# ramanathanlab/distllm

Hardware: NVIDIA H100
Metric: embedded chunks/sec @512-tok (higher is better)
Workload: dtype bf16

## Files before the change

distllm_b200/csrc/attention.cuh:

```cuda
#pragma once

#include "common.cuh"

namespace b2e {

constexpr int AT_KC = 64;
constexpr float AT_MASKED = -3.0e38f;

template <int D, int V>
struct AtCfg {
  static constexpr int COLS = D < 64 ? D : 64;
  static constexpr int ROW_BYTES = 2 * COLS;
  static constexpr int BOX = 64 * ROW_BYTES;
  static constexpr int NB = D / COLS;
  static constexpr int NWG = (V & 64) ? 4 : 2;
  static constexpr int QT = 64 * NWG;
  static constexpr int THREADS = 128 * NWG + (NWG == 4 ? 128 : 32);
  static constexpr int CONSUMER_REGS = 112, PRODUCER_REGS = 24;
  static constexpr int STAGES = D == 128 ? 3 : 4;
  static constexpr int Q_BYTES = NWG * NB * BOX;
  static constexpr int STAGE_BYTES = 2 * NB * BOX;
  static_assert(D == 32 || D == 64 || D == 128, "head_dim");
  static constexpr int BAR = Q_BYTES + STAGES * STAGE_BYTES;
  static constexpr int SMEM_BYTES = BAR + 256 + 1024;
  static_assert(SMEM_BYTES <= 232448, "shared memory");
};

__device__ long long* g_att_clock = nullptr;

__device__ __forceinline__ float poly_exp2(float x) {
  x = fmaxf(x, -126.0f);
  const float n = rintf(x);
  const float f = x - n;
  float p = fmaf(f, 9.6181291e-3f, 5.5504109e-2f);
  p = fmaf(f, p, 2.4022651e-1f);
  p = fmaf(f, p, 6.9314718e-1f);
  p = fmaf(f, p, 1.0f);
  return __int_as_float(__float_as_int(p) + (static_cast<int>(n) << 23));
}

template <int ROW_BYTES>
__device__ __forceinline__ uint64_t at_box_desc(uint32_t saddr) {
  if constexpr (ROW_BYTES == 128) return make_smem_desc_sw128(saddr);
  else return make_smem_desc_sw64(saddr);
}

__global__ void attn_prep_kernel(const int64_t* __restrict__ mask, float* __restrict__ bias,
                                 int* __restrict__ kv_chunks, int* __restrict__ plain_chunks, int B, int S,
                                 int S_pad) {
  const int b = blockIdx.x * (blockDim.x >> 5) + (threadIdx.x >> 5);
  if (b >= B) return;
  const int lane = threadIdx.x & 31;
  int last = 0;
  int first_off = S_pad;
  for (int j = lane; j < S_pad; j += 32) {
    float v = -INFINITY;
    bool on = false;
    if (j < S) {
      on = mask[static_cast<size_t>(b) * S + j] != 0;
      v = on ? 0.0f : AT_MASKED;
      if (on) last = j + 1;
    }
    if (!on) first_off = min(first_off, j);
    bias[static_cast<size_t>(b) * S_pad + j] = v;
  }
#pragma unroll
  for (int o = 16; o > 0; o >>= 1) {
    last = max(last, __shfl_xor_sync(0xffffffffu, last, o));
    first_off = min(first_off, __shfl_xor_sync(0xffffffffu, first_off, o));
  }
  if (lane == 0) {
    kv_chunks[b] = last > 0 ? (last + AT_KC - 1) / AT_KC : S_pad / AT_KC;
    plain_chunks[b] = first_off / AT_KC;
  }
}

template <int D, int MODE, int V>
__global__ void __launch_bounds__(AtCfg<D, V>::THREADS, 1)
attention_kernel(const __grid_constant__ CUtensorMap tm, const __grid_constant__ CUtensorMap tm_ctx,
                 const float* __restrict__ bias, const int* __restrict__ kv_chunks,
                 const int* __restrict__ plain_chunks, int B, int S, int S_pad, int heads, int kv_heads, int window,
                 float scale_log2e, const int* __restrict__ seq_cu, const int* __restrict__ seq_len,
                 h16* __restrict__ ctx) {
  using Cfg = AtCfg<D, V>;
  constexpr int NB = Cfg::NB;
  constexpr int COLS = Cfg::COLS, BOX = Cfg::BOX, RB = Cfg::ROW_BYTES;
  constexpr int NWG = Cfg::NWG;
  constexpr int POLY = (V >> 2) & 3;
  constexpr bool EPI_ROLE = (V & 128) != 0;
  constexpr bool STAMPS = (V & 256) != 0;
  static_assert(MODE == 0 || (V & ~(64 | 128)) == 0, "windowed / causal attention: warpgroups and epilogue role only");
  const int h = blockIdx.x % heads;
  const int b = (blockIdx.x / heads) % B;
  const int tile = static_cast<int>(gridDim.x / (heads * B)) - 1 - static_cast<int>(blockIdx.x / (heads * B));
  const int row0 = seq_cu != nullptr ? __ldg(seq_cu + b) : b * S;
  const int len = seq_len != nullptr ? __ldg(seq_len + b) : S;
  const int q0 = tile * Cfg::QT;
  if (q0 >= len) return;
  const int kvc = __ldg(kv_chunks + b);
  const int np = (V & 1) ? __ldg(plain_chunks + b) : 0;
  int lo = 0, hi = kvc;
  if (MODE == 1) {
    lo = max(0, q0 - window) / AT_KC;
    hi = min(kvc, (q0 + Cfg::QT - 1 + window) / AT_KC + 1);
  } else if (MODE == 2) {
    lo = window > 0 ? max(0, q0 - window + 1) / AT_KC : 0;
    hi = min(kvc, (q0 + Cfg::QT - 1) / AT_KC + 1);
  }
  if (lo >= hi) lo = hi - 1;

  extern __shared__ uint8_t smem_raw[];
  const uint32_t sb = (smem_u32(smem_raw) + 1023u) & ~1023u;
  const uint32_t q_bar = sb + Cfg::BAR;
  const uint32_t full_bar = q_bar + 8;
  const uint32_t empty_bar = full_bar + 8u * Cfg::STAGES;
  const uint32_t out_bar = empty_bar + 8u * Cfg::STAGES;
  const int warp = threadIdx.x >> 5;
  const int kvh = h / (heads / kv_heads);
  const int qcol = h * D, kcol = (heads + kvh) * D, vcol = (heads + kv_heads + kvh) * D;

  if (threadIdx.x == 0) {
    mbar_init(q_bar, 1);
    for (int s = 0; s < Cfg::STAGES; ++s) {
      mbar_init(full_bar + 8u * s, 1);
      mbar_init(empty_bar + 8u * s, NWG);
    }
    for (int w = 0; w < NWG; ++w) mbar_init(out_bar + 8u * w, 1);
    mbar_fence_init();
  }
  __syncthreads();

  if (warp >= 4 * NWG) {
    if constexpr (NWG == 4) asm volatile("setmaxnreg.dec.sync.aligned.u32 %0;" ::"n"(Cfg::PRODUCER_REGS));
    if (warp == 4 * NWG && elect_one()) {
      tma_prefetch_desc(&tm);
      mbar_expect_tx(q_bar, Cfg::Q_BYTES);
#pragma unroll
      for (int w = 0; w < NWG; ++w)
#pragma unroll
        for (int x = 0; x < NB; ++x)
          tma_load_2d(sb + (w * NB + x) * BOX, &tm, q_bar, qcol + COLS * x, row0 + q0 + 64 * w);
      int stage = 0;
      uint32_t phase = 0;
      for (int c = lo; c < hi; ++c) {
        mbar_wait(empty_bar + 8u * stage, phase ^ 1u);
        const uint32_t fb = full_bar + 8u * stage;
        const uint32_t dst = sb + Cfg::Q_BYTES + stage * Cfg::STAGE_BYTES;
        mbar_expect_tx(fb, Cfg::STAGE_BYTES);
#pragma unroll
        for (int x = 0; x < NB; ++x) {
          tma_load_2d(dst + x * BOX, &tm, fb, kcol + COLS * x, row0 + c * AT_KC);
          tma_load_2d(dst + (NB + x) * BOX, &tm, fb, vcol + COLS * x, row0 + c * AT_KC);
        }
        if (++stage == Cfg::STAGES) { stage = 0; phase ^= 1u; }
      }
      if constexpr (EPI_ROLE) {
        for (int w = 0; w < NWG; ++w) {
          mbar_wait(out_bar + 8u * w, 0);
          if (q0 + 64 * w + 64 > len) continue;
#pragma unroll
          for (int x = 0; x < NB; ++x)
            tma_store_2d(&tm_ctx, sb + (w * NB + x) * BOX, h * D + COLS * x, row0 + q0 + 64 * w);
        }
        tma_store_commit();
        tma_store_wait_all();
      }
    }
    return;
  }

  if constexpr (NWG == 4) asm volatile("setmaxnreg.inc.sync.aligned.u32 %0;" ::"n"(Cfg::CONSUMER_REGS));
  const int wg = warp >> 2;
  const int t = threadIdx.x & 127;
  const int quad = t & 3;
  const int qr = q0 + 64 * wg + 16 * (t >> 5) + ((t & 31) >> 2);
  const float* brow = bias + static_cast<size_t>(b) * S_pad;
  const uint32_t q_addr = sb + wg * NB * BOX;
  long long* clk = nullptr;
  int n_stamp = 0;
  if (STAMPS && blockIdx.x == 0 && threadIdx.x == 0) clk = g_att_clock;

  constexpr int OG = COLS / 8;
  float o[NB][4 * OG];
#pragma unroll
  for (int x = 0; x < NB; ++x)
#pragma unroll
    for (int i = 0; i < 4 * OG; ++i) o[x][i] = 0.0f;
  float m[2] = {-INFINITY, -INFINITY}, l[2] = {0.0f, 0.0f};

  mbar_wait(q_bar, 0);
  int stage = 0;
  uint32_t phase = 0;
  for (int c = lo; c < hi; ++c) {
    mbar_wait(full_bar + 8u * stage, phase);
    const uint32_t k_addr = sb + Cfg::Q_BYTES + stage * Cfg::STAGE_BYTES;
    const uint32_t v_addr = k_addr + NB * BOX;
    float s[32];
#pragma unroll
    for (int i = 0; i < 32; ++i) s[i] = 0.0f;
    wgmma_fence();
    constexpr int KB = COLS / 16;
#pragma unroll
    for (int kk = 0; kk < D / 16; ++kk)
      wgmma_64x64_ss<0>(s, at_box_desc<RB>(q_addr + (kk / KB) * BOX) + 2u * (kk % KB),
                        at_box_desc<RB>(k_addr + (kk / KB) * BOX) + 2u * (kk % KB), kk != 0);
    wgmma_commit();
    wgmma_wait<0>();
    reg_fence(s);
    if (STAMPS && clk != nullptr && n_stamp < 256) {
      clk[n_stamp] = clock64();
      clk[256 + n_stamp++] = 2 * c + 1;
    }

    const int kbase = c * AT_KC + 2 * quad;
    const bool plain = MODE == 0 && (V & 1) && c < np;
#pragma unroll
    for (int j = 0; j < 8; ++j) {
      const float2 bz = plain ? make_float2(0.0f, 0.0f) : *reinterpret_cast<const float2*>(brow + kbase + 8 * j);
#pragma unroll
      for (int e = 0; e < 4; ++e) {
        const int key = kbase + 8 * j + (e & 1);
        const int q = qr + 8 * (e >> 1);
        float x = fmaf(s[4 * j + e], scale_log2e, (e & 1) ? bz.y : bz.x);
        if (MODE == 1 && abs(q - key) > window) x = AT_MASKED;
        if (MODE == 2 && (key > q || (window > 0 && q - key >= window))) x = AT_MASKED;
        s[4 * j + e] = x;
      }
    }
    float alpha[2];
#pragma unroll
    for (int hf = 0; hf < 2; ++hf) {
      float mx = m[hf];
#pragma unroll
      for (int j = 0; j < 8; ++j) mx = fmaxf(mx, fmaxf(s[4 * j + 2 * hf], s[4 * j + 2 * hf + 1]));
      mx = fmaxf(mx, __shfl_xor_sync(0xffffffffu, mx, 1));
      mx = fmaxf(mx, __shfl_xor_sync(0xffffffffu, mx, 2));
      alpha[hf] = fast_exp2(m[hf] - mx);
      m[hf] = mx;
    }
    uint32_t p[4][4];
    float rs[2] = {0.0f, 0.0f};
#pragma unroll
    for (int j = 0; j < 8; ++j) {
#pragma unroll
      for (int hf = 0; hf < 2; ++hf) {
        const float x0 = s[4 * j + 2 * hf] - m[hf], x1 = s[4 * j + 2 * hf + 1] - m[hf];
        const int k0 = (2 * (j & 1) + hf) * 2;
        const float p0 = (k0 % 4) < POLY ? poly_exp2(x0) : fast_exp2(x0);
        const float p1 = ((k0 + 1) % 4) < POLY ? poly_exp2(x1) : fast_exp2(x1);
        rs[hf] += p0 + p1;
        p[j >> 1][(j & 1) * 2 + hf] = pack_h16x2(p0, p1);
      }
    }
#pragma unroll
    for (int hf = 0; hf < 2; ++hf) l[hf] = l[hf] * alpha[hf] + rs[hf];
#pragma unroll
    for (int x = 0; x < NB; ++x)
#pragma unroll
      for (int j = 0; j < OG; ++j) {
        o[x][4 * j + 0] *= alpha[0];
        o[x][4 * j + 1] *= alpha[0];
        o[x][4 * j + 2] *= alpha[1];
        o[x][4 * j + 3] *= alpha[1];
      }

#pragma unroll
    for (int x = 0; x < NB; ++x) reg_fence(o[x]);
    wgmma_fence();
#pragma unroll
    for (int kc = 0; kc < 4; ++kc)
#pragma unroll
      for (int x = 0; x < NB; ++x) {
        if constexpr (COLS == 64) wgmma_64x64_rs_tb(o[x], p[kc], make_smem_desc_sw128(v_addr + x * BOX + kc * 16 * 128));
        else wgmma_64x32_rs_tb(o[x], p[kc], make_smem_desc_sw64(v_addr + x * BOX + kc * 16 * 64));
      }
    wgmma_commit();
    wgmma_wait<0>();
#pragma unroll
    for (int x = 0; x < NB; ++x) reg_fence(o[x]);
    if (STAMPS && clk != nullptr && n_stamp < 256) {
      clk[n_stamp] = clock64();
      clk[256 + n_stamp++] = 2 * c + 2;
    }
    if (t == 0) mbar_arrive(empty_bar + 8u * stage);
    if (++stage == Cfg::STAGES) { stage = 0; phase ^= 1u; }
  }

  const bool staged = EPI_ROLE && q0 + 64 * wg + 64 <= len;
#pragma unroll
  for (int hf = 0; hf < 2; ++hf) {
    float tot = l[hf];
    tot += __shfl_xor_sync(0xffffffffu, tot, 1);
    tot += __shfl_xor_sync(0xffffffffu, tot, 2);
    const float inv = 1.0f / tot;
    const int q = qr + 8 * hf;
    if (staged) {
      const int r = q - q0 - 64 * wg;
      const int swz = RB == 128 ? (r & 7) : ((r >> 1) & 3);
#pragma unroll
      for (int x = 0; x < NB; ++x)
#pragma unroll
        for (int j = 0; j < OG; ++j) {
          const uint32_t off = r * RB + ((j ^ swz) << 4) + 4 * quad;
          *reinterpret_cast<uint32_t*>(smem_raw + (q_addr - smem_u32(smem_raw)) + x * BOX + off) =
              pack_h16x2(o[x][4 * j + 2 * hf] * inv, o[x][4 * j + 2 * hf + 1] * inv);
        }
      continue;
    }
    if (q >= len) continue;
    h16* orow = ctx + static_cast<size_t>(row0 + q) * (heads * D) + h * D + 2 * quad;
#pragma unroll
    for (int x = 0; x < NB; ++x)
#pragma unroll
      for (int j = 0; j < OG; ++j)
        *reinterpret_cast<uint32_t*>(orow + COLS * x + 8 * j) =
            pack_h16x2(o[x][4 * j + 2 * hf] * inv, o[x][4 * j + 2 * hf + 1] * inv);
  }
  if constexpr (EPI_ROLE) {
    fence_proxy_async_smem();
    asm volatile("bar.sync %0, 128;" ::"r"(1 + wg) : "memory");
    if (t == 0) mbar_arrive(out_bar + 8u * wg);
  }
}

}
```

distllm_b200/csrc/b2e_api.cu:

```cuda
#include "../../include/b2e.h"
#include "../../include/b2e_debug.h"

#include <cuda.h>
#include <cuda_runtime.h>

#include <cstdarg>
#include <cstdio>
#include <cstdlib>
#include <cstring>
#include <string>
#include <utility>
#include <vector>

#include "attention.cuh"
#include "binsearch.cuh"
#include "common.cuh"
#include "gemm.cuh"
#include "mistral_ops.cuh"
#include "pack.cuh"
#include "rowops.cuh"
#include "topk.cuh"
#include "topk_tc.cuh"

using namespace b2e;
// ... 178 lines not shown
  CUtensorMap tm;
  const float* absmax = nullptr;
  int bn = GEMM_BN;
};

int make_gemm_w(GemmW* w, const void* base, const float* absmax, uint64_t rows, uint64_t cols, int epi) {
  w->absmax = absmax;
  w->bn = gemm_bn((int)rows, epi, absmax != nullptr);
  return absmax ? make_tmap_codes(&w->tm, base, rows, cols / 2) : make_tmap_h16(&w->tm, base, rows, cols, w->bn);
}

template <int EPI>
int launch_gemm_epi(const CUtensorMap& ta, const GemmW& wb, void* out, const float* bias,
                    const h16* resid, int M, int N, int K, cudaStream_t st, const int* m_dev) {
  auto kern = gemm_h16_wgmma_kernel<EPI>;
  int smem = GemmPlan<false>::SMEM_BYTES;
  if (N % wb.bn != 0) return fail(B2E_ERR_INVALID, "gemm: N=%d is not a multiple of its W map's tile width %d", N, wb.bn);
  if (wb.absmax) {
    kern = gemm_h16_wgmma_kernel<EPI, false, true>;
    smem = GemmPlan<true>::SMEM_BYTES;
  } else if (wb.bn == 192) {
    if constexpr (epi_is_glu(EPI)) {
      return fail(B2E_ERR_INVALID, "gemm: the gated epilogues run 128-wide tiles only");
    } else {
      kern = gemm_h16_wgmma_kernel<EPI, false, false, 192>;
      smem = GemmPlan<false, 192>::SMEM_BYTES;
      if constexpr (EPI == EPI_BIAS || EPI == EPI_BIAS_GELU)
        if (g_gemm_profiling) kern = gemm_h16_wgmma_kernel<EPI, true, false, 192>;
    }
  } else if constexpr (EPI == EPI_BIAS || EPI == EPI_BIAS_GELU) {
    if (g_gemm_profiling) kern = gemm_h16_wgmma_kernel<EPI, true>;
  }
  int rc = ensure_smem_attr(kern, smem);
  if (rc) return rc;
  DeviceInfo dev;
  if ((rc = current_device_info(&dev))) return rc;
  const long long tiles = (long long)(N / wb.bn) * ((M + GEMM_BM - 1) / GEMM_BM);
  if (tiles > 0x7fffffffLL) return fail(B2E_ERR_INVALID, "gemm: %lld output tiles exceed one grid", tiles);
  CUtensorMap tm_out;
  if ((rc = make_tmap_h16(&tm_out, out, M, epi_is_glu(EPI) ? N / 2 : N, GEMM_BM))) return rc;
  const unsigned grid = (unsigned)(tiles < dev.sms ? tiles : dev.sms);
  kern<<<grid, GEMM_THREADS, smem, st>>>(ta, wb.tm, tm_out, static_cast<h16*>(out), bias, resid, M, N, K, m_dev,
                                         wb.absmax);
  CUDA_TRY(cudaGetLastError());
  return B2E_OK;
}

int launch_gemm(const CUtensorMap& ta, const GemmW& tb, void* out, const float* bias,
                const void* resid, int M, int N, int K, int epi, cudaStream_t st, const int* m_dev = nullptr) {
  const h16* r = static_cast<const h16*>(resid);
  switch (epi) {
    case B2E_EPI_BIAS: return launch_gemm_epi<EPI_BIAS>(ta, tb, out, bias, r, M, N, K, st, m_dev);
    case B2E_EPI_BIAS_GELU: return launch_gemm_epi<EPI_BIAS_GELU>(ta, tb, out, bias, r, M, N, K, st, m_dev);
    case B2E_EPI_BIAS_RESID: return launch_gemm_epi<EPI_BIAS_RESID>(ta, tb, out, bias, r, M, N, K, st, m_dev);
    case B2E_EPI_SWIGLU: return launch_gemm_epi<EPI_SWIGLU>(ta, tb, out, bias, r, M, N, K, st, m_dev);
    case B2E_EPI_GEGLU: return launch_gemm_epi<EPI_GEGLU>(ta, tb, out, bias, r, M, N, K, st, m_dev);
  }
  return fail(B2E_ERR_INVALID, "unknown epilogue %d", epi);
}

template <typename T>
struct DevBuf {
  T* p = nullptr;
  size_t cap = 0;
  operator T*() const { return p; }
  int grow(size_t n, uint64_t& gen, bool zero = false) {
    if (n <= cap) return B2E_OK;
    ++gen;
    release();
    CUDA_TRY(cudaMalloc(&p, n * sizeof(T)));
    if (zero) CUDA_TRY(cudaMemset(p, 0, n * sizeof(T)));
    cap = n;
    return B2E_OK;
  }
  void release() {
    cudaFree(p);
    p = nullptr;
    cap = 0;
  }
};

struct DeviceScratch {
  int device = -1;
  uint64_t gen = 0;
};

template <typename Scratch>
int follow_device(Scratch& s) {
  int dev = 0;
  CUDA_TRY(cudaGetDevice(&dev));
  if (dev != s.device) {
    s.release();
    s.device = dev;
    ++s.gen;
  }
  return B2E_OK;
}

struct AttnScratch : DeviceScratch {
  DevBuf<float> bias;
  DevBuf<int> kv_chunks;
  DevBuf<int> plain_chunks;
  int ensure(int B, int S_pad) {
    int rc;
    if ((rc = follow_device(*this)) || (rc = bias.grow((size_t)B * S_pad, gen)) || (rc = kv_chunks.grow(B, gen)) ||
        (rc = plain_chunks.grow(B, gen)))
      return rc;
    return B2E_OK;
  }
  void release() {
    bias.release();
    kv_chunks.release();
    plain_chunks.release();
  }
};

inline int attn_s_pad(int S) { return (S + AT_KC - 1) / AT_KC * AT_KC; }

int attention_prepare(AttnScratch& sc, const int64_t* mask, int B, int S, cudaStream_t st) {
  int rc;
  const int S_pad = attn_s_pad(S);
  if ((rc = sc.ensure(B, S_pad))) return rc;
  attn_prep_kernel<<<(B + 7) / 8, 256, 0, st>>>(mask, sc.bias, sc.kv_chunks, sc.plain_chunks, B, S, S_pad);
  CUDA_TRY(cudaGetLastError());
  return B2E_OK;
}

struct SeqLayout {
  const int* cu = nullptr;
  const int* len = nullptr;
  const int* t_real = nullptr;
  const int* tok_src = nullptr;
};

struct PackBuffers : DeviceScratch {
  DevBuf<int> len_raw, ok, len;
  DevBuf<int> cu;
  DevBuf<int> t_real;
  DevBuf<int> src;
  int ensure(int B, size_t tokens) {
    int rc;
    if ((rc = follow_device(*this)) || (rc = len_raw.grow(B, gen)) || (rc = ok.grow(B, gen)) ||
        (rc = len.grow(B, gen)) || (rc = cu.grow((size_t)B + 1, gen)) || (rc = t_real.grow(2, gen)) ||
        (rc = src.grow(tokens, gen)))
      return rc;
    return B2E_OK;
  }
  void release() {
    len_raw.release(); ok.release(); len.release(); cu.release(); t_real.release(); src.release();
  }
};

template <int D, int MODE, int V>
int launch_attention_kernel(const CUtensorMap& tm, const AttnScratch& sc, void* ctx, int B, int S, int heads,
                            int kv_heads, int window, cudaStream_t st, const SeqLayout& lay) {
  using Cfg = AtCfg<D, V>;
  auto kern = attention_kernel<D, MODE, V>;
  int rc = ensure_smem_attr(kern, Cfg::SMEM_BYTES);
  if (rc) return rc;
  CUtensorMap tm_ctx = {};
  if ((V & 128) && (rc = make_tmap_h16(&tm_ctx, ctx, (uint64_t)B * S, (uint64_t)heads * D, 64, Cfg::COLS))) return rc;
  const float scale_log2e = 1.4426950408889634f / sqrtf(static_cast<float>(D));
  const long long ctas = (long long)heads * B * ((S + Cfg::QT - 1) / Cfg::QT);
  if (ctas > 0x7fffffffLL)
    return fail(B2E_ERR_INVALID, "attention: %lld CTAs (heads=%d B=%d S=%d) exceed one grid", ctas, heads, B, S);
  kern<<<(unsigned)ctas, Cfg::THREADS, Cfg::SMEM_BYTES, st>>>(tm, tm_ctx, sc.bias, sc.kv_chunks, sc.plain_chunks, B, S,
                                                    attn_s_pad(S), heads, kv_heads, window, scale_log2e, lay.cu,
                                                    lay.len, static_cast<h16*>(ctx));
  CUDA_TRY(cudaGetLastError());
  return B2E_OK;
}

constexpr int AT_DEFAULT_VARIANT = 193;
int g_att3_variant = -1;
inline int att3_variant() {
  if (g_att3_variant < 0) {
    const char* e = getenv("B2E_ATT3");
    g_att3_variant = e ? atoi(e) : AT_DEFAULT_VARIANT;
  }
  return g_att3_variant;
}

int launch_attention(const CUtensorMap& tkv, const AttnScratch& sc, void* ctx, int B, int S, int heads,
                     cudaStream_t st, int window = 0, const SeqLayout& lay = SeqLayout()) {
  const int v = att3_variant();
#define B2E_ATT(MODE, V) launch_attention_kernel<64, MODE, V>(tkv, sc, ctx, B, S, heads, heads, window, st, lay)
  if (window > 0) {
    switch (v & 192) {
      case 0: return B2E_ATT(1, 0);
      case 64: return B2E_ATT(1, 64);
      case 128: return B2E_ATT(1, 128);
      case 192: return B2E_ATT(1, 192);
    }
    return fail(B2E_ERR_INVALID, "windowed attention: variant %d has no instantiation (bits 6-7 of the variant pick "
                "0, 64, 128 or 192)", v);
  }
  switch (v) {
    case 0: return B2E_ATT(0, 0);
    case 1: return B2E_ATT(0, 1);
    case 5: return B2E_ATT(0, 5);
    case 64: return B2E_ATT(0, 64);
    case 65: return B2E_ATT(0, 65);
    case 69: return B2E_ATT(0, 69);
    case 193: return B2E_ATT(0, 193);
    case 261: return B2E_ATT(0, 261);
    case 321: return B2E_ATT(0, 321);
  }
#undef B2E_ATT
  return fail(B2E_ERR_INVALID, "attention variant %d is not instantiated (0,1,5,64,65,69,193,261,321)", v);
}

int launch_attention_causal_d128(const void* qkv, AttnScratch& sc, void* ctx, int B, int S, int heads,
                                 int kv_heads, int window, cudaStream_t st, const SeqLayout& lay = SeqLayout()) {
  CUtensorMap tm;
  const int rc = make_tmap_h16(&tm, qkv, (uint64_t)B * S, (uint64_t)(heads + 2 * kv_heads) * 128, AT_KC);
  if (rc) return rc;
  return launch_attention_kernel<128, 2, 0>(tm, sc, ctx, B, S, heads, kv_heads, window, st, lay);
}

constexpr int AT_D32_VARIANT = 1;

int launch_attention_bidir(const CUtensorMap& tqkv, const AttnScratch& sc, void* ctx, int B, int S, int heads,
                           int head_dim, cudaStream_t st, const SeqLayout& lay = SeqLayout()) {
  if (head_dim == 32)
    return launch_attention_kernel<32, 0, AT_D32_VARIANT>(tqkv, sc, ctx, B, S, heads, heads, 0, st, lay);
  return launch_attention(tqkv, sc, ctx, B, S, heads, st, 0, lay);
}

#define DISPATCH_H(H, CALL)                                         \
  switch (H) {                                                      \
    case 256: { constexpr int HW = 256; CALL; break; }              \
    case 384: { constexpr int HW = 384; CALL; break; }              \
    case 512: { constexpr int HW = 512; CALL; break; }              \
    case 640: { constexpr int HW = 640; CALL; break; }              \
    case 768: { constexpr int HW = 768; CALL; break; }              \
    case 1024: { constexpr int HW = 1024; CALL; break; }            \
    case 1280: { constexpr int HW = 1280; CALL; break; }            \
    case 2048: { constexpr int HW = 2048; CALL; break; }            \
    case 2560: { constexpr int HW = 2560; CALL; break; }            \
    case 4096: { constexpr int HW = 4096; CALL; break; }            \
    default: return fail(B2E_ERR_INVALID, "hidden size %d not supported (need 256*{1,2,3,4,5,8,10,16}, 384 or 640)", (H)); \
  }

inline int row_blocks(int rows) { return (rows + ROW_WARPS - 1) / ROW_WARPS; }

int check_h(int H) {
  if (H == 384 || H == 640) return B2E_OK;
  if (H % 256 != 0) return fail(B2E_ERR_INVALID, "hidden size %d must be a multiple of 256, or 384 or 640", H);
  switch (H / 256) {
    case 1: case 2: case 3: case 4: case 5: case 8: case 10: case 16: return B2E_OK;
  }
  return fail(B2E_ERR_UNSUPPORTED, "hidden size %d not supported (built: 256 x {1,2,3,4,5,8,10,16}, 384, 640)", H);
}

struct PoolScratch : DeviceScratch {
  DevBuf<int> seq_len;
  DevBuf<int> kill;
  DevBuf<int> idx;
  DevBuf<float> w;
  DevBuf<float> count;
  DevBuf<float> part;
  int ensure(int B, int S, size_t part_elems) {
    int rc;
    if ((rc = follow_device(*this)) || (rc = seq_len.grow(B, gen)) || (rc = kill.grow(S, gen)) ||
        (rc = idx.grow(B, gen)) || (rc = w.grow((size_t)B * S, gen)) || (rc = count.grow(B, gen)) ||
        (rc = part.grow(part_elems, gen)))
      return rc;
    return B2E_OK;
  }
  void release() {
    seq_len.release(); kill.release(); idx.release(); w.release(); count.release(); part.release();
  }
};

inline int pool_nsplit(int S) {
  int n = (S + 63) / 64;
  return n < 1 ? 1 : (n > 16 ? 16 : n);
}

int launch_pool_weights(PoolScratch& ps, int64_t* mask, int B, int S, int pool_kind, int mutate,
                        cudaStream_t st) {
  seq_len_kernel<<<(B + 7) / 8, 256, 0, st>>>(mask, ps.seq_len, B, S);
  CUDA_TRY(cudaMemsetAsync(ps.kill, 0, sizeof(int) * S, st));
  kill_columns_kernel<<<(B + 255) / 256, 256, 0, st>>>(ps.seq_len, ps.kill, B, S);
  pool_weights_kernel<<<(B + 7) / 8, 256, 0, st>>>(mask, ps.seq_len, ps.kill, ps.w, ps.count, B, S,
                                                    pool_kind == B2E_POOL_MEAN_REF ? 1 : 0, mutate);
  CUDA_TRY(cudaGetLastError());
  return B2E_OK;
}

int launch_finalize(PoolScratch& ps, float* out, int B, int H, int nsplit, int l2, int round_mode,
                    cudaStream_t st) {
  pool_finalize_kernel<<<B, 256, (H + 32) * sizeof(float), st>>>(ps.part, ps.count, out, H, nsplit,
                                                                 l2, round_mode);
  CUDA_TRY(cudaGetLastError());
  return B2E_OK;
}

struct DeviceGuard {
  int prev = -1;
  DeviceGuard() {
    if (cudaGetDevice(&prev) != cudaSuccess) {
      cudaGetLastError();
      prev = -1;
    }
  }
  ~DeviceGuard() {
    if (prev >= 0) cudaSetDevice(prev);
  }
};

thread_local PoolScratch g_pool_scratch;
thread_local AttnScratch g_attn_scratch;
thread_local PackBuffers g_pack_scratch;

}

inline bool is_decoder(int arch) { return arch == B2E_ARCH_MISTRAL || arch == B2E_ARCH_QWEN3; }

namespace {
enum FinalNorm {
  NORM_POST_LN,
  NORM_ADD_LN,
  NORM_ADD_RMS,
};

using TrunkFn = int (*)(B2EEncoder* e, const int64_t* ids, const int64_t* mask, const int64_t* types, int B, int S,
                        cudaStream_t st, const SeqLayout& lay);

struct Family {
  int lead, stride;
  int wqkv, wo, w1, w2;
  bool w1_gated;
  int w1_epi;
  FinalNorm norm;
  int norm_g, norm_b;
  TrunkFn trunk;
};
const Family* family(int arch);
}

struct B2EEncoder {
  B2EModelDesc desc;
  const Family* fam = nullptr;
  int full_layers = 0;
  std::vector<const void*> w;
  int device = 0;
  int sms = 0;
  DevBuf<h16> hidden, qkv, ctx, tmp, ffn;
  DevBuf<float> xres, tok_scale;
  PoolScratch pool;
  AttnScratch attn;
  PackBuffers pack;
  std::vector<GemmW> tm_wqkv, tm_wo, tm_w1, tm_w2;
  DevBuf<int64_t> stage_in;
  DevBuf<float> stage_out;
  cudaStream_t own_stream = nullptr;
  float *rope_cos = nullptr, *rope_sin = nullptr;
  float *rope_cos2 = nullptr, *rope_sin2 = nullptr;

  const void* slot(int l, int k) const { return w[fam->lead + fam->stride * l + k]; }
  const float* final_norm(int k) const {
// ... 1255 lines not shown
```

Before: 5007.

## Add ping-pong warpgroup attention kernel for head_dim 64 and make it default

Adds a new FlashAttention-3 style kernel for head_dim 64. Two consumer warpgroups each own 128 query rows and alternate wgmma issue through named barriers. Inside each turn, the S=QK^T GEMM for the next chunk overlaps the PV GEMM for the previous chunk, so softmax runs while the tensor cores stay busy. It uses 8 KV stages, 240 consumer registers and a TMA store epilogue, and it becomes the default variant (705). The risks are register pressure and barrier ordering in the ping-pong schedule, and the larger per-CTA query tile may lower parallelism at short sequence lengths.

Measured after the change: 5050, median of 6. About the same (+0.9%).

```diff
diff --git a/distllm_b200/csrc/attention.cuh b/distllm_b200/csrc/attention.cuh
--- a/distllm_b200/csrc/attention.cuh
+++ b/distllm_b200/csrc/attention.cuh
@@ -323,4 +323,266 @@
   }
 }
 
-}
+constexpr int AT_BAR_TURN = 1, AT_BAR_EPI = 3;
+
+struct AtPingPongCfg {
+  static constexpr int COLS = 64;
+  static constexpr int BOX = 64 * 2 * COLS;
+  static constexpr int NWG = 2;
+  static constexpr int QT = 128 * NWG;
+  static constexpr int THREADS = 128 * NWG + 128;
+  static constexpr int CONSUMER_REGS = 240, PRODUCER_REGS = 24;
+  static constexpr int STAGES = 8;
+  static constexpr int Q_BYTES = 2 * NWG * BOX;
+  static constexpr int STAGE_BYTES = 2 * BOX;
+  static constexpr int BAR = Q_BYTES + STAGES * STAGE_BYTES;
+  static constexpr int SMEM_BYTES = BAR + 256 + 1024;
+  static_assert(SMEM_BYTES <= 232448, "shared memory");
+};
+
+__device__ __forceinline__ void at_softmax_block(float (&s)[32], const float2 (&bz)[8], float scale_log2e,
+                                                 float (&m)[2], float (&l)[2], float (&alpha)[2],
+                                                 uint32_t (&p)[4][4]) {
+#pragma unroll
+  for (int j = 0; j < 8; ++j)
+#pragma unroll
+    for (int e = 0; e < 4; ++e) s[4 * j + e] = fmaf(s[4 * j + e], scale_log2e, (e & 1) ? bz[j].y : bz[j].x);
+#pragma unroll
+  for (int hf = 0; hf < 2; ++hf) {
+    float mx = m[hf];
+#pragma unroll
+    for (int j = 0; j < 8; ++j) mx = fmaxf(mx, fmaxf(s[4 * j + 2 * hf], s[4 * j + 2 * hf + 1]));
+    mx = fmaxf(mx, __shfl_xor_sync(0xffffffffu, mx, 1));
+    mx = fmaxf(mx, __shfl_xor_sync(0xffffffffu, mx, 2));
+    alpha[hf] = fast_exp2(m[hf] - mx);
+    m[hf] = mx;
+  }
+  float rs[2] = {0.0f, 0.0f};
+#pragma unroll
+  for (int j = 0; j < 8; ++j)
+#pragma unroll
+    for (int hf = 0; hf < 2; ++hf) {
+      const float p0 = fast_exp2(s[4 * j + 2 * hf] - m[hf]), p1 = fast_exp2(s[4 * j + 2 * hf + 1] - m[hf]);
+      rs[hf] += p0 + p1;
+      p[j >> 1][(j & 1) * 2 + hf] = pack_h16x2(p0, p1);
+    }
+#pragma unroll
+  for (int hf = 0; hf < 2; ++hf) l[hf] = l[hf] * alpha[hf] + rs[hf];
+}
+
+template <int V>
+__global__ void __launch_bounds__(AtPingPongCfg::THREADS, 1)
+pingpong_attention_kernel(const __grid_constant__ CUtensorMap tm, const __grid_constant__ CUtensorMap tm_ctx,
+                          const float* __restrict__ bias, const int* __restrict__ kv_chunks,
+                          const int* __restrict__ plain_chunks, int B, int S, int S_pad, int heads, int kv_heads,
+                          int window, float scale_log2e, const int* __restrict__ seq_cu,
+                          const int* __restrict__ seq_len, h16* __restrict__ ctx) {
+  using Cfg = AtPingPongCfg;
+  constexpr int BOX = Cfg::BOX, NWG = Cfg::NWG, D = 64;
+  static_assert(V & 512, "ping-pong variants have bit 9 set");
+  const int tiles = static_cast<int>(gridDim.x / (heads * B));
+  const int tile = static_cast<int>(blockIdx.x % tiles);
+  const int h = static_cast<int>(blockIdx.x / tiles) % heads;
+  const int b = static_cast<int>(blockIdx.x / (tiles * heads));
+  const int row0 = seq_cu != nullptr ? __ldg(seq_cu + b) : b * S;
+  const int len = seq_len != nullptr ? __ldg(seq_len + b) : S;
+  const int q0 = tile * Cfg::QT;
+  if (q0 >= len) return;
+  const int lo = 0, hi = __ldg(kv_chunks + b);
+  const int np = (V & 1) ? __ldg(plain_chunks + b) : 0;
+
+  extern __shared__ uint8_t smem_raw[];
+  const uint32_t sb = (smem_u32(smem_raw) + 1023u) & ~1023u;
+  const uint32_t q_bar = sb + Cfg::BAR;
+  const uint32_t full_bar = q_bar + 8;
+  const uint32_t empty_bar = full_bar + 8u * Cfg::STAGES;
+  const int warp = threadIdx.x >> 5;
+  const int kvh = h / (heads / kv_heads);
+  const int qcol = h * D, kcol = (heads + kvh) * D, vcol = (heads + kv_heads + kvh) * D;
+
+  if (threadIdx.x == 0) {
+    mbar_init(q_bar, 1);
+    for (int s = 0; s < Cfg::STAGES; ++s) {
+      mbar_init(full_bar + 8u * s, 1);
+      mbar_init(empty_bar + 8u * s, NWG);
+    }
+    mbar_fence_init();
+  }
+  __syncthreads();
+
+  if (warp >= 4 * NWG) {
+    asm volatile("setmaxnreg.dec.sync.aligned.u32 %0;" ::"n"(Cfg::PRODUCER_REGS));
+    if (warp == 4 * NWG && elect_one()) {
+      tma_prefetch_desc(&tm);
+      mbar_expect_tx(q_bar, Cfg::Q_BYTES);
+#pragma unroll
+      for (int x = 0; x < 2 * NWG; ++x) tma_load_2d(sb + x * BOX, &tm, q_bar, qcol, row0 + q0 + 64 * x);
+      int stage = 0;
+      uint32_t phase = 0;
+      for (int c = lo; c < hi; ++c) {
+        mbar_wait(empty_bar + 8u * stage, phase ^ 1u);
+        const uint32_t fb = full_bar + 8u * stage;
+        const uint32_t dst = sb + Cfg::Q_BYTES + stage * Cfg::STAGE_BYTES;
+        mbar_expect_tx(fb, Cfg::STAGE_BYTES);
+        tma_load_2d(dst, &tm, fb, kcol, row0 + c * AT_KC);
+        tma_load_2d(dst + BOX, &tm, fb, vcol, row0 + c * AT_KC);
+        if (++stage == Cfg::STAGES) { stage = 0; phase ^= 1u; }
+      }
+    }
+    return;
+  }
+
+  asm volatile("setmaxnreg.inc.sync.aligned.u32 %0;" ::"n"(Cfg::CONSUMER_REGS));
+  const int wg = warp >> 2;
+  const int t = threadIdx.x & 127;
+  const int quad = t & 3;
+  const int r_lo = 16 * (t >> 5) + ((t & 31) >> 2);
+  const int wrow = q0 + 128 * wg;
+  const float* brow = bias + static_cast<size_t>(b) * S_pad;
+  const uint32_t q_addr = sb + 2 * wg * BOX;
+
+  float o[2][32], s[2][32];
+#pragma unroll
+  for (int i = 0; i < 32; ++i) o[0][i] = o[1][i] = s[0][i] = s[1][i] = 0.0f;
+  float m[2][2] = {{-INFINITY, -INFINITY}, {-INFINITY, -INFINITY}}, l[2][2] = {{0.0f, 0.0f}, {0.0f, 0.0f}};
+  uint32_t pa[2][4][4], pb[2][4][4];
+
+  auto issue_s = [&](uint32_t k_addr) {
+#pragma unroll
+    for (int kk = 0; kk < D / 16; ++kk)
+#pragma unroll
+      for (int bl = 0; bl < 2; ++bl)
+        wgmma_64x64_ss<0>(s[bl], make_smem_desc_sw128(q_addr + bl * BOX) + 2u * kk,
+                          make_smem_desc_sw128(k_addr) + 2u * kk, kk != 0);
+  };
+  auto issue_pv = [&](const uint32_t (&p)[2][4][4], uint32_t v_addr) {
+#pragma unroll
+    for (int kc = 0; kc < 4; ++kc)
+#pragma unroll
+      for (int bl = 0; bl < 2; ++bl) wgmma_64x64_rs_tb(o[bl], p[bl][kc], make_smem_desc_sw128(v_addr + kc * 16 * 128));
+  };
+  auto load_bias = [&](int c, float2 (&bz)[8]) {
+    const bool plain = (V & 1) && c < np;
+    const int kbase = c * AT_KC + 2 * quad;
+#pragma unroll
+    for (int j = 0; j < 8; ++j)
+      bz[j] = plain ? make_float2(0.0f, 0.0f) : *reinterpret_cast<const float2*>(brow + kbase + 8 * j);
+  };
+  const uint32_t kv0 = sb + Cfg::Q_BYTES;
+
+  mbar_wait(q_bar, 0);
+  float alpha[2][2];
+  {
+    float2 bz[8];
+    load_bias(lo, bz);
+    mbar_wait(full_bar, 0);
+    if (wg == 1) named_bar_sync(AT_BAR_TURN + 1, 256);
+    wgmma_fence();
+    issue_s(kv0);
+    wgmma_commit();
+    named_bar_arrive(AT_BAR_TURN + (wg ^ 1), 256);
+    wgmma_wait<0>();
+    reg_fence(s[0]);
+    reg_fence(s[1]);
+#pragma unroll
+    for (int bl = 0; bl < 2; ++bl) at_softmax_block(s[bl], bz, scale_log2e, m[bl], l[bl], alpha[bl], pa[bl]);
+  }
+  static_assert(Cfg::STAGES > 1, "chunk lo + 1 is in stage 1");
+  int stage = 1, prev = 0;
+  uint32_t phase = 0;
+  auto turn = [&](int c, const uint32_t (&in)[2][4][4], uint32_t (&out)[2][4][4]) {
+    float2 bz[8];
+    load_bias(c, bz);
+    mbar_wait(full_bar + 8u * stage, phase);
+    named_bar_sync(AT_BAR_TURN + wg, 256);
+    reg_fence(o[0]);
+    reg_fence(o[1]);
+    wgmma_fence();
+    issue_s(kv0 + stage * Cfg::STAGE_BYTES);
+    wgmma_commit();
+    issue_pv(in, kv0 + prev * Cfg::STAGE_BYTES + BOX);
+    wgmma_commit();
+    named_bar_arrive(AT_BAR_TURN + (wg ^ 1), 256);
+    wgmma_wait<1>();
+    reg_fence(s[0]);
+    reg_fence(s[1]);
+#pragma unroll
+    for (int bl = 0; bl < 2; ++bl) at_softmax_block(s[bl], bz, scale_log2e, m[bl], l[bl], alpha[bl], out[bl]);
+    wgmma_wait<0>();
+    reg_fence(o[0]);
+    reg_fence(o[1]);
+    if (t == 0) mbar_arrive(empty_bar + 8u * prev);
+#pragma unroll
+    for (int bl = 0; bl < 2; ++bl)
+#pragma unroll
+      for (int j = 0; j < 8; ++j) {
+        o[bl][4 * j + 0] *= alpha[bl][0];
+        o[bl][4 * j + 1] *= alpha[bl][0];
+        o[bl][4 * j + 2] *= alpha[bl][1];
+        o[bl][4 * j + 3] *= alpha[bl][1];
+      }
+    prev = stage;
+    if (++stage == Cfg::STAGES) { stage = 0; phase ^= 1u; }
+  };
+  auto last_turn = [&](const uint32_t (&in)[2][4][4]) {
+    named_bar_sync(AT_BAR_TURN + wg, 256);
+    reg_fence(o[0]);
+    reg_fence(o[1]);
+    wgmma_fence();
+    issue_pv(in, kv0 + prev * Cfg::STAGE_BYTES + BOX);
+    wgmma_commit();
+    if (wg == 0) named_bar_arrive(AT_BAR_TURN + 1, 256);
+    wgmma_wait<0>();
+    reg_fence(o[0]);
+    reg_fence(o[1]);
+  };
+  int c = lo + 1;
+  for (; c + 1 < hi; c += 2) {
+    turn(c, pa, pb);
+    turn(c + 1, pb, pa);
+  }
+  if (c < hi) {
+    turn(c, pa, pb);
+    last_turn(pb);
+  } else {
+    last_turn(pa);
+  }
+
+#pragma unroll
+  for (int bl = 0; bl < 2; ++bl) {
+    const int r0 = wrow + 64 * bl;
+    const bool staged = r0 + 64 <= len;
+#pragma unroll
+    for (int hf = 0; hf < 2; ++hf) {
+      float tot = l[bl][hf];
+      tot += __shfl_xor_sync(0xffffffffu, tot, 1);
+      tot += __shfl_xor_sync(0xffffffffu, tot, 2);
+      const float inv = 1.0f / tot;
+      const int r = r_lo + 8 * hf;
+      if (staged) {
+#pragma unroll
+        for (int j = 0; j < 8; ++j)
+          st_shared_u32(q_addr + bl * BOX + r * 128 + ((j ^ (r & 7)) << 4) + 4 * quad,
+                        pack_h16x2(o[bl][4 * j + 2 * hf] * inv, o[bl][4 * j + 2 * hf + 1] * inv));
+        continue;
+      }
+      if (r0 + r >= len) continue;
+      h16* orow = ctx + static_cast<size_t>(row0 + r0 + r) * (heads * D) + h * D + 2 * quad;
+#pragma unroll
+      for (int j = 0; j < 8; ++j)
+        *reinterpret_cast<uint32_t*>(orow + 8 * j) =
+            pack_h16x2(o[bl][4 * j + 2 * hf] * inv, o[bl][4 * j + 2 * hf + 1] * inv);
+    }
+  }
+  fence_proxy_async_smem();
+  named_bar_sync(AT_BAR_EPI + wg, 128);
+  if (t == 0) {
+#pragma unroll
+    for (int bl = 0; bl < 2; ++bl)
+      if (wrow + 64 * bl + 64 <= len) tma_store_2d(&tm_ctx, q_addr + bl * BOX, h * D, row0 + wrow + 64 * bl);
+    tma_store_commit();
+    tma_store_wait_read<0>();
+  }
+}
+
+}
diff --git a/distllm_b200/csrc/b2e_api.cu b/distllm_b200/csrc/b2e_api.cu
--- a/distllm_b200/csrc/b2e_api.cu
+++ b/distllm_b200/csrc/b2e_api.cu
@@ -354,10 +354,20 @@
 };
 
 template <int D, int MODE, int V>
+constexpr auto attention_kernel_of() {
+  if constexpr ((V & 512) != 0) {
+    static_assert(D == 64 && MODE == 0, "the ping-pong kernel is head_dim 64, MODE 0");
+    return pingpong_attention_kernel<V>;
+  } else {
+    return attention_kernel<D, MODE, V>;
+  }
+}
+
+template <int D, int MODE, int V>
 int launch_attention_kernel(const CUtensorMap& tm, const AttnScratch& sc, void* ctx, int B, int S, int heads,
                             int kv_heads, int window, cudaStream_t st, const SeqLayout& lay) {
-  using Cfg = AtCfg<D, V>;
-  auto kern = attention_kernel<D, MODE, V>;
+  using Cfg = std::conditional_t<(V & 512) != 0, AtPingPongCfg, AtCfg<D, V>>;
+  auto kern = attention_kernel_of<D, MODE, V>();
   int rc = ensure_smem_attr(kern, Cfg::SMEM_BYTES);
   if (rc) return rc;
   CUtensorMap tm_ctx = {};
@@ -373,7 +383,7 @@
   return B2E_OK;
 }
 
-constexpr int AT_DEFAULT_VARIANT = 193;
+constexpr int AT_DEFAULT_VARIANT = 705;
 int g_att3_variant = -1;
 inline int att3_variant() {
   if (g_att3_variant < 0) {
@@ -407,9 +417,10 @@
     case 193: return B2E_ATT(0, 193);
     case 261: return B2E_ATT(0, 261);
     case 321: return B2E_ATT(0, 321);
+    case 705: return B2E_ATT(0, 705);
   }
 #undef B2E_ATT
-  return fail(B2E_ERR_INVALID, "attention variant %d is not instantiated (0,1,5,64,65,69,193,261,321)", v);
+  return fail(B2E_ERR_INVALID, "attention variant %d is not instantiated (0,1,5,64,65,69,193,261,321,705)", v);
 }
 
 int launch_attention_causal_d128(const void* qkv, AttnScratch& sc, void* ctx, int B, int S, int heads,
```

## Overlap next QK wgmma with previous PV wgmma in attention consumer loop

Applied to the files above, without the earlier changes.

Adds an OVERLAP attention variant (bit 512) where each consumer turn issues the QK^T wgmma for the next KV chunk and the PV wgmma for the previous chunk back-to-back. It waits only on the QK group before computing the row max, so tensor-core work overlaps with the softmax. It also deepens the KV pipeline to 5 stages for this variant and makes it the default (705 = 193|512). The cost is more shared memory, a P register array that lives across iterations, and more complex stage/release bookkeeping.

Result: no change. 4983 before, 5030 after, median of 6 (+1.0%).

```diff
diff --git a/distllm_b200/csrc/attention.cuh b/distllm_b200/csrc/attention.cuh
--- a/distllm_b200/csrc/attention.cuh
+++ b/distllm_b200/csrc/attention.cuh
@@ -17,7 +17,7 @@
   static constexpr int QT = 64 * NWG;
   static constexpr int THREADS = 128 * NWG + (NWG == 4 ? 128 : 32);
   static constexpr int CONSUMER_REGS = 112, PRODUCER_REGS = 24;
-  static constexpr int STAGES = D == 128 ? 3 : 4;
+  static constexpr int STAGES = D == 128 ? 3 : (V & 512) ? 5 : 4;
   static constexpr int Q_BYTES = NWG * NB * BOX;
   static constexpr int STAGE_BYTES = 2 * NB * BOX;
   static_assert(D == 32 || D == 64 || D == 128, "head_dim");
@@ -89,6 +89,7 @@
   constexpr int POLY = (V >> 2) & 3;
   constexpr bool EPI_ROLE = (V & 128) != 0;
   constexpr bool STAMPS = (V & 256) != 0;
+  constexpr bool OVERLAP = (V & 512) != 0;
   static_assert(MODE == 0 || (V & ~(64 | 128)) == 0, "windowed / causal attention: warpgroups and epilogue role only");
   const int h = blockIdx.x % heads;
   const int b = (blockIdx.x / heads) % B;
@@ -178,7 +179,14 @@
   const uint32_t q_addr = sb + wg * NB * BOX;
   long long* clk = nullptr;
   int n_stamp = 0;
-  if (STAMPS && blockIdx.x == 0 && threadIdx.x == 0) clk = g_att_clock;
+  if (STAMPS && g_att_clock != nullptr && blockIdx.x == 0 && (threadIdx.x == 0 || (OVERLAP && threadIdx.x == 256)))
+    clk = g_att_clock + 512 * (wg >> 1);
+  auto stamp = [&](int event) {
+    if (STAMPS && clk != nullptr && n_stamp < 256) {
+      clk[n_stamp] = clock64();
+      clk[256 + n_stamp++] = event;
+    }
+  };
 
   constexpr int OG = COLS / 8;
   float o[NB][4 * OG];
@@ -188,30 +196,24 @@
     for (int i = 0; i < 4 * OG; ++i) o[x][i] = 0.0f;
   float m[2] = {-INFINITY, -INFINITY}, l[2] = {0.0f, 0.0f};
 
-  mbar_wait(q_bar, 0);
-  int stage = 0;
-  uint32_t phase = 0;
-  for (int c = lo; c < hi; ++c) {
-    mbar_wait(full_bar + 8u * stage, phase);
-    const uint32_t k_addr = sb + Cfg::Q_BYTES + stage * Cfg::STAGE_BYTES;
-    const uint32_t v_addr = k_addr + NB * BOX;
-    float s[32];
-#pragma unroll
-    for (int i = 0; i < 32; ++i) s[i] = 0.0f;
-    wgmma_fence();
+  auto issue_qk = [&](float (&s)[32], uint32_t k_addr) {
     constexpr int KB = COLS / 16;
 #pragma unroll
     for (int kk = 0; kk < D / 16; ++kk)
       wgmma_64x64_ss<0>(s, at_box_desc<RB>(q_addr + (kk / KB) * BOX) + 2u * (kk % KB),
                         at_box_desc<RB>(k_addr + (kk / KB) * BOX) + 2u * (kk % KB), kk != 0);
-    wgmma_commit();
-    wgmma_wait<0>();
-    reg_fence(s);
-    if (STAMPS && clk != nullptr && n_stamp < 256) {
-      clk[n_stamp] = clock64();
-      clk[256 + n_stamp++] = 2 * c + 1;
-    }
-
+  };
+  auto issue_pv = [&](const uint32_t (&p)[4][4], uint32_t v_addr) {
+#pragma unroll
+    for (int kc = 0; kc < 4; ++kc)
+#pragma unroll
+      for (int x = 0; x < NB; ++x) {
+        if constexpr (COLS == 64) wgmma_64x64_rs_tb(o[x], p[kc], make_smem_desc_sw128(v_addr + x * BOX + kc * 16 * 128));
+        else wgmma_64x32_rs_tb(o[x], p[kc], make_smem_desc_sw64(v_addr + x * BOX + kc * 16 * 64));
+      }
+  };
+
+  auto softmax_max = [&](float (&s)[32], int c, float (&alpha)[2]) {
     const int kbase = c * AT_KC + 2 * quad;
     const bool plain = MODE == 0 && (V & 1) && c < np;
 #pragma unroll
@@ -227,7 +229,6 @@
         s[4 * j + e] = x;
       }
     }
-    float alpha[2];
 #pragma unroll
     for (int hf = 0; hf < 2; ++hf) {
       float mx = m[hf];
@@ -238,7 +239,8 @@
       alpha[hf] = fast_exp2(m[hf] - mx);
       m[hf] = mx;
     }
-    uint32_t p[4][4];
+  };
+  auto softmax_exp = [&](float (&s)[32], const float (&alpha)[2], uint32_t (&p)[4][4]) {
     float rs[2] = {0.0f, 0.0f};
 #pragma unroll
     for (int j = 0; j < 8; ++j) {
@@ -263,27 +265,85 @@
         o[x][4 * j + 2] *= alpha[1];
         o[x][4 * j + 3] *= alpha[1];
       }
-
-#pragma unroll
-    for (int x = 0; x < NB; ++x) reg_fence(o[x]);
-    wgmma_fence();
-#pragma unroll
-    for (int kc = 0; kc < 4; ++kc)
-#pragma unroll
-      for (int x = 0; x < NB; ++x) {
-        if constexpr (COLS == 64) wgmma_64x64_rs_tb(o[x], p[kc], make_smem_desc_sw128(v_addr + x * BOX + kc * 16 * 128));
-        else wgmma_64x32_rs_tb(o[x], p[kc], make_smem_desc_sw64(v_addr + x * BOX + kc * 16 * 64));
-      }
-    wgmma_commit();
-    wgmma_wait<0>();
-#pragma unroll
-    for (int x = 0; x < NB; ++x) reg_fence(o[x]);
-    if (STAMPS && clk != nullptr && n_stamp < 256) {
-      clk[n_stamp] = clock64();
-      clk[256 + n_stamp++] = 2 * c + 2;
-    }
-    if (t == 0) mbar_arrive(empty_bar + 8u * stage);
-    if (++stage == Cfg::STAGES) { stage = 0; phase ^= 1u; }
+  };
+
+  if constexpr (OVERLAP) stamp(1);
+  mbar_wait(q_bar, 0);
+  int stage = 0;
+  uint32_t phase = 0;
+  if constexpr (!OVERLAP) {
+    for (int c = lo; c < hi; ++c) {
+      mbar_wait(full_bar + 8u * stage, phase);
+      const uint32_t k_addr = sb + Cfg::Q_BYTES + stage * Cfg::STAGE_BYTES;
+      float s[32];
+#pragma unroll
+      for (int i = 0; i < 32; ++i) s[i] = 0.0f;
+      wgmma_fence();
+      issue_qk(s, k_addr);
+      wgmma_commit();
+      wgmma_wait<0>();
+      reg_fence(s);
+      stamp(2 * c + 1);
+      uint32_t p[4][4];
+      float alpha[2];
+      softmax_max(s, c, alpha);
+      softmax_exp(s, alpha, p);
+#pragma unroll
+      for (int x = 0; x < NB; ++x) reg_fence(o[x]);
+      wgmma_fence();
+      issue_pv(p, k_addr + NB * BOX);
+      wgmma_commit();
+      wgmma_wait<0>();
+#pragma unroll
+      for (int x = 0; x < NB; ++x) reg_fence(o[x]);
+      stamp(2 * c + 2);
+      if (t == 0) mbar_arrive(empty_bar + 8u * stage);
+      if (++stage == Cfg::STAGES) { stage = 0; phase ^= 1u; }
+    }
+  } else {
+    uint32_t p[4][4];
+    int pstage = 0;
+    auto turn = [&](int i, bool pv, bool qk) {
+      const uint32_t k_addr = sb + Cfg::Q_BYTES + stage * Cfg::STAGE_BYTES;
+      if (qk) mbar_wait(full_bar + 8u * stage, phase);
+      float s[32];
+#pragma unroll
+      for (int j = 0; j < 32; ++j) s[j] = 0.0f;
+#pragma unroll
+      for (int x = 0; x < NB; ++x) reg_fence(o[x]);
+      wgmma_fence();
+      if (qk) {
+        issue_qk(s, k_addr);
+        wgmma_commit();
+      }
+      if (pv) {
+        issue_pv(p, sb + Cfg::Q_BYTES + pstage * Cfg::STAGE_BYTES + NB * BOX);
+        wgmma_commit();
+      }
+      stamp(4 + 4 * i);
+      float alpha[2];
+      if (qk) {
+        if (pv) wgmma_wait<1>();
+        else wgmma_wait<0>();
+        reg_fence(s);
+        stamp(4 + 4 * i + 1);
+        softmax_max(s, lo + i, alpha);
+      }
+      wgmma_wait<0>();
+#pragma unroll
+      for (int x = 0; x < NB; ++x) reg_fence(o[x]);
+      stamp(4 + 4 * i + 2);
+      if (pv && t == 0) mbar_arrive(empty_bar + 8u * pstage);
+      if (qk) {
+        softmax_exp(s, alpha, p);
+        pstage = stage;
+        if (++stage == Cfg::STAGES) { stage = 0; phase ^= 1u; }
+      }
+    };
+    const int turns = hi - lo + 1;
+    turn(0, false, true);
+    for (int i = 1; i + 1 < turns; ++i) turn(i, true, true);
+    turn(turns - 1, true, false);
   }
 
   const bool staged = EPI_ROLE && q0 + 64 * wg + 64 <= len;
@@ -321,6 +381,7 @@
     asm volatile("bar.sync %0, 128;" ::"r"(1 + wg) : "memory");
     if (t == 0) mbar_arrive(out_bar + 8u * wg);
   }
-}
-
-}
+  if constexpr (OVERLAP) stamp(2);
+}
+
+}
diff --git a/distllm_b200/csrc/b2e_api.cu b/distllm_b200/csrc/b2e_api.cu
--- a/distllm_b200/csrc/b2e_api.cu
+++ b/distllm_b200/csrc/b2e_api.cu
@@ -373,7 +373,7 @@
   return B2E_OK;
 }
 
-constexpr int AT_DEFAULT_VARIANT = 193;
+constexpr int AT_DEFAULT_VARIANT = 705;
 int g_att3_variant = -1;
 inline int att3_variant() {
   if (g_att3_variant < 0) {
@@ -407,9 +407,11 @@
     case 193: return B2E_ATT(0, 193);
     case 261: return B2E_ATT(0, 261);
     case 321: return B2E_ATT(0, 321);
+    case 705: return B2E_ATT(0, 705);
+    case 961: return B2E_ATT(0, 961);
   }
 #undef B2E_ATT
-  return fail(B2E_ERR_INVALID, "attention variant %d is not instantiated (0,1,5,64,65,69,193,261,321)", v);
+  return fail(B2E_ERR_INVALID, "attention variant %d is not instantiated (0,1,5,64,65,69,193,261,321,705,961)", v);
 }
 
 int launch_attention_causal_d128(const void* qkv, AttnScratch& sc, void* ctx, int B, int S, int heads,
```
